# telosnetwork/plonky2_goldibear

Measured on AMD Instinct MI355X. Metric: proofs/s, higher is better.
Workload: dtype u64; 1 GPU; prove(): 2^20-row Goldilocks dummy circuit (2^19+1 NoopGates), standard_recursion_config_gl with num_challenges=3, Poseidon-12, witness in page-locked host memory, handed over every step -> proof bytes (198432 B); field=goldilocks, log_n=20, cap_height=4, proofs_in_flight_per_gpu=1, witness=in page-locked host memory, handed over every step

## Files before the change

plonky2_goldibear_amd/csrc/field_traits.hpp:

```cpp
#pragma once
#include "bb_field.hpp"
#include "gl_field.hpp"

#define GB_HD __host__ __device__ __forceinline__
#if defined(__HIP_DEVICE_COMPILE__)
#define GB_DEV_OR_HOST(dev, host) dev
#else
#define GB_DEV_OR_HOST(dev, host) host
#endif

namespace gbk {

typedef unsigned long long u64;
typedef unsigned int u32;

struct GlF {
    typedef u64 T;
    typedef gl::ext2 E;
    static constexpr u32 D = 2, H = 4, SPONGE_W = 12, ORDER_BITS = 64, TWO_ADICITY = 32, TAG = 0;
    static constexpr u64 ORDER = gl::P;
    static GB_HD T zero() { return 0; }
    static GB_HD T one() { return 1; }
    static GB_HD T enc(u64 canonical) { return canonical; }
    static GB_HD u64 dec(T x) { return x; }
    static GB_HD T reduce_word(T x) { return x >= gl::P ? x - gl::P : x; }
    static GB_HD T add(T a, T b) { return gl::add(a, b); }
    static GB_HD T sub(T a, T b) { return gl::sub(a, b); }
    static GB_HD T mul(T a, T b) { return gl::mul(a, b); }
    static GB_HD T mul_lazy(T a, T b) {
        u32 r0, r1, hl, hh;
        gl::mul_limbs(a, b, r0, r1, hl, hh);
        return gl::fold128(r0, r1, hl, hh);
    }
    static GB_HD T add_lazy(T a, T b) { return gl::add(a, b); }
    static GB_HD T cform(T c) { return gl::to_mont_slow(c); }
    static GB_HD T chain_one(u32 len) {
        constexpr unsigned __int128 R = gl::EPS;
        struct Tab { u64 v[17]; };
        constexpr Tab t = [] {
            Tab x{};
            unsigned __int128 a = 1;
            for (int i = 0; i < 17; i++) { x.v[i] = (u64)a; a = a * R % gl::P; }
            return x;
        }();
        return t.v[len];
    }
    static GB_HD T mul_chain(T acc, T f) { return gl::mul_mont_lazy(acc, f); }
    static GB_HD T mulc(T x, T c_form) { return gl::mul_mont(x, c_form); }
    typedef T Acc;
    static GB_HD Acc acc_from(T x) { return x; }
    static GB_HD void acc_mac2(Acc& a0, Acc& a1, T term, T c0, T c1) {
        a0 = add(a0, mulc(term, c0));
        a1 = add(a1, mulc(term, c1));
    }
    static GB_HD void acc_mac(Acc& a, T term, T c) { a = add(a, mulc(term, c)); }
    static GB_HD T acc_finish(Acc a) { return a; }
    static GB_HD T inv(T a) { return gl::inv(a); }
    static GB_HD T pow(T a, u64 e) { return gl::pow(a, e); }
    static GB_HD T generator() { return gl::GENERATOR; }
    static GB_HD T two_adic_generator(u32 bits) { return gl::two_adic_generator(bits); }
    static GB_HD T ext_w() { return 7; }
    static GB_HD E ezero() { return gl::e2(0); }
    static GB_HD E efrom(T x) { return gl::e2(x); }
    static GB_HD E eadd(E a, E b) { return gl::add(a, b); }
    static GB_HD E esub(E a, E b) { return gl::sub(a, b); }
    static GB_HD E emul(E a, E b) { return gl::mul(a, b); }
    static GB_HD E escale(E a, T s) { return gl::scale(a, s); }
    static GB_HD E einv(E a) { return gl::inv(a); }
    static GB_HD T coord(const E& e, u32 k) { return k ? e.c1 : e.c0; }
    static GB_HD void set_coord(E& e, u32 k, T v) { if (k) e.c1 = v; else e.c0 = v; }
};

struct bb_ext4 {
    u32 c[4];
};

struct BbF {
    typedef u32 T;
    typedef bb_ext4 E;
    static constexpr u32 D = 4, H = 8, SPONGE_W = 16, ORDER_BITS = 31, TWO_ADICITY = 27, TAG = 1;
    static constexpr u64 ORDER = bb::P;
    static constexpr u32 W_MONT = (u32)((11ull << 32) % bb::P);
    static GB_HD T zero() { return 0; }
    static GB_HD T one() { return bb::R1; }
    static GB_HD T enc(u64 canonical) { return bb::to_mont((u32)canonical); }
    static GB_HD u64 dec(T x) { return bb::from_mont(x); }
    static GB_HD T reduce_word(T x) {
        x = x >= 2 * bb::P ? x - 2 * bb::P : x;
        return x >= bb::P ? x - bb::P : x;
    }
    static GB_HD T add(T a, T b) { return bb::add(a, b); }
    static GB_HD T sub(T a, T b) { return bb::sub(a, b); }
    static GB_HD T mul(T a, T b) { return bb::mul(a, b); }
    static GB_HD T mul_lazy(T a, T b) { return bb::mul(a, b); }
    static GB_HD T add_lazy(T a, T b) { return a + b; }
    static GB_HD T cform(T c) { return c; }
    static GB_HD T mulc(T x, T c_form) { return bb::mul(x, c_form); }
    static GB_HD T chain_one(u32) { return bb::R1; }
    static GB_HD T mul_chain(T acc, T f) { return bb::mul(acc, f); }
    struct Acc {
        u64 lo;
        u32 hi;
    };
    static GB_HD Acc acc_from(T x) { return Acc{(u64)x << 32, 0u}; }
    static GB_HD void acc_mac2(Acc& a0, Acc& a1, T term, T c0, T c1) {
#if defined(__HIP_DEVICE_COMPILE__)
        u64 k0, k1;
        asm("v_mad_u64_u32 %0, %4, %6, %7, %0\n\t"
            "v_mad_u64_u32 %2, %5, %6, %8, %2\n\t"
            "s_nop 0\n\t"
            "v_addc_co_u32_e64 %1, %4, 0, %1, %4\n\t"
            "v_addc_co_u32_e64 %3, %5, 0, %3, %5"
            : "+v"(a0.lo), "+v"(a0.hi), "+v"(a1.lo), "+v"(a1.hi), "=&s"(k0), "=&s"(k1)
            : "v"(term), "s"(c0), "s"(c1));
#else
        acc_mac(a0, term, c0);
        acc_mac(a1, term, c1);
#endif
    }
    static GB_HD void acc_mac(Acc& a, T term, T c) {
        const u64 p = (u64)term * c, s = a.lo + p;
        a.hi += s < p;
        a.lo = s;
    }
    static GB_HD T acc_finish(Acc a) {
        const T top = bb::mul(a.hi, bb::R2);
        const T mid = bb::mul((u32)(a.lo >> 32), bb::R1);
        const T low = bb::reduce((u64)(u32)a.lo);
        return bb::add(bb::add(top, mid), low);
    }
    static GB_HD T inv(T a) { return bb::inv(a); }
    static GB_HD T pow(T a, u64 e) { return bb::pow(a, e); }
    static GB_HD T generator() { return bb::to_mont(bb::GENERATOR); }
    static GB_HD T two_adic_generator(u32 bits) { return bb::two_adic_generator(bits); }
    static GB_HD T ext_w() { return W_MONT; }
    static GB_HD E ezero() { return E{{0, 0, 0, 0}}; }
    static GB_HD E efrom(T x) { return E{{x, 0, 0, 0}}; }
    static GB_HD E eadd(E a, E b) { return E{{bb::add(a.c[0], b.c[0]), bb::add(a.c[1], b.c[1]), bb::add(a.c[2], b.c[2]), bb::add(a.c[3], b.c[3])}}; }
    static GB_HD E esub(E a, E b) { return E{{bb::sub(a.c[0], b.c[0]), bb::sub(a.c[1], b.c[1]), bb::sub(a.c[2], b.c[2]), bb::sub(a.c[3], b.c[3])}}; }
    static GB_HD E emul(E a, E b) {
        using bb::add; using bb::mul;
        u32 lo0 = mul(a.c[0], b.c[0]);
        u32 lo1 = add(mul(a.c[0], b.c[1]), mul(a.c[1], b.c[0]));
        u32 lo2 = add(add(mul(a.c[0], b.c[2]), mul(a.c[1], b.c[1])), mul(a.c[2], b.c[0]));
        u32 lo3 = add(add(mul(a.c[0], b.c[3]), mul(a.c[1], b.c[2])), add(mul(a.c[2], b.c[1]), mul(a.c[3], b.c[0])));
        u32 hi0 = add(add(mul(a.c[1], b.c[3]), mul(a.c[2], b.c[2])), mul(a.c[3], b.c[1]));
        u32 hi1 = add(mul(a.c[2], b.c[3]), mul(a.c[3], b.c[2]));
        u32 hi2 = mul(a.c[3], b.c[3]);
        return E{{add(lo0, mul(W_MONT, hi0)), add(lo1, mul(W_MONT, hi1)), add(lo2, mul(W_MONT, hi2)), lo3}};
    }
    static GB_HD E escale(E a, T s) { return E{{bb::mul(a.c[0], s), bb::mul(a.c[1], s), bb::mul(a.c[2], s), bb::mul(a.c[3], s)}}; }
    static __host__ __device__ inline E einv(E a) {
        using bb::add; using bb::sub; using bb::mul;
        const u32 a0 = a.c[0], a1 = a.c[1], a2 = a.c[2], a3 = a.c[3];
        u32 b2_0 = add(mul(a1, a1), mul(W_MONT, mul(a3, a3))), b2_1 = mul(add(a1, a1), a3);
        u32 c0 = sub(add(mul(a0, a0), mul(W_MONT, mul(a2, a2))), mul(W_MONT, b2_1));
        u32 c1 = sub(mul(add(a0, a0), a2), b2_0);
        u32 ninv = bb::inv(sub(mul(c0, c0), mul(W_MONT, mul(c1, c1))));
        u32 d0 = mul(c0, ninv), d1 = mul(bb::neg(c1), ninv);
        u32 ad0 = add(mul(a0, d0), mul(W_MONT, mul(a2, d1))), ad1 = add(mul(a0, d1), mul(a2, d0));
        u32 bd0 = add(mul(a1, d0), mul(W_MONT, mul(a3, d1))), bd1 = add(mul(a1, d1), mul(a3, d0));
        return E{{ad0, bb::neg(bd0), ad1, bb::neg(bd1)}};
    }
    static GB_HD T coord(const E& e, u32 k) { return e.c[k]; }
    static GB_HD void set_coord(E& e, u32 k, T v) { e.c[k] = v; }
};

template <class F>
__host__ __device__ inline typename F::E epow(typename F::E b, u64 e) {
    typename F::E r = F::efrom(F::one());
    while (e) {
        if (e & 1) r = F::emul(r, b);
        b = F::emul(b, b);
        e >>= 1;
    }
    return r;
}
template <class F>
__host__ __device__ inline bool eis_one(const typename F::E& e) {
    bool ok = F::coord(e, 0) == F::one();
    for (u32 k = 1; k < F::D; k++) ok = ok && F::coord(e, k) == F::zero();
    return ok;
}

}
```

plonky2_goldibear_amd/csrc/kernels_prover.hip:

```cpp
#include "kernels.hpp"
#include "poseidon2_bb.hpp"
#include "poseidon_gl_grouped.hpp"
#include "sponge.hpp"

namespace gbk {

__device__ __forceinline__ u32 brev32(u32 x, u32 bits) { return bits ? (__brev(x) >> (32 - bits)) : 0; }

template <class F>
__device__ __forceinline__ typename F::T pow_split(const PowTab<F>& t, u64 e) {
    typename F::T lo = t.lo[e & ((1u << t.lo_bits) - 1)];
    u64 h = e >> t.lo_bits;
    return h ? F::mul(lo, t.hi[h]) : lo;
}
template <class F>
__device__ __forceinline__ typename F::E pow_split(const ExtPowTab<F>& t, u64 e) {
    typename F::E l = t.lo[e & ((1u << t.lo_bits) - 1)];
    u64 h = e >> t.lo_bits;
    return h ? F::emul(l, t.hi[h]) : l;
}


template <class F>
__global__ __launch_bounds__(256) void k_zs_quotients(ZsParams<F> p, const typename F::T* __restrict__ witness,
                                                      const typename F::T* __restrict__ sigma, const typename F::T* __restrict__ k_is,
                                                      typename F::T* __restrict__ q, u32* __restrict__ err) {
    typedef typename F::T T;
    const u32 nb = (u32)((((size_t)1 << p.log_n) + 255) >> 8), L = blockIdx.x;
    u32 rb, ch;
    if ((nb & 7) == 0) {
        const u32 group = L / (8 * p.num_challenges), in = L % (8 * p.num_challenges);
        rb = group * 8 + (in & 7);
        ch = in >> 3;
    } else {
        rb = L % nb;
        ch = L / nb;
    }
    const u32 row = rb * 256 + threadIdx.x;
    const size_t n = (size_t)1 << p.log_n;
    if (row >= n) return;
    const T beta = p.betas[ch], gamma = p.gammas[ch];
    const T bx = F::mul(beta, pow_split(p.w_n, row));
    T N[MAX_CHUNKS], Dn[MAX_CHUNKS];
    for (u32 m = 0; m < p.nchunks; m++) {
        T np = F::one(), dp = F::one();
        const u32 j1 = min((m + 1) * p.chunk, p.num_routed);
        for (u32 j = m * p.chunk; j < j1; j++) {
            T w = witness[(size_t)j * n + row];
            const T wg = F::add(w, gamma);
            T num = F::add_lazy(wg, F::mul(bx, k_is[j]));
            T den = F::add_lazy(wg, F::mul(beta, sigma[(size_t)j * n + row]));
            np = F::mul_lazy(np, num);
            dp = F::mul_lazy(dp, den);
        }
        N[m] = np;
        Dn[m] = dp;
    }
    T pref[MAX_CHUNKS];
    T acc = F::one();
    for (u32 m = 0; m < p.nchunks; m++) {
        pref[m] = acc;
        acc = F::mul(acc, Dn[m]);
    }
    if (acc == F::zero()) {
        atomicOr(err, 1u);
        return;
    }
    T inv_run = F::inv(acc);
    for (u32 m = p.nchunks; m-- > 0;) {
        T dinv = F::mul(inv_run, pref[m]);
        inv_run = F::mul(inv_run, Dn[m]);
        q[((size_t)ch * p.nchunks + m) * n + row] = F::mul(N[m], dinv);
    }
}

template <class F>
__global__ __launch_bounds__(256) void k_zs_scan_local(ZsParams<F> p, const typename F::T* __restrict__ q,
                                                       typename F::T* __restrict__ zloc, typename F::T* __restrict__ totals) {
    typedef typename F::T T;
    __shared__ T sh[256];
    const size_t n = (size_t)1 << p.log_n;
    const u32 ch = blockIdx.y;
    const size_t row0 = (size_t)blockIdx.x * 1024 + threadIdx.x * 4;
    T r[4];
#pragma unroll
    for (int k = 0; k < 4; k++) {
        T v = F::one();
        if (row0 + k < n)
            for (u32 m = 0; m < p.nchunks; m++) v = F::mul(v, q[((size_t)ch * p.nchunks + m) * n + row0 + k]);
        r[k] = v;
    }
    T mine = F::mul(F::mul(r[0], r[1]), F::mul(r[2], r[3]));
    sh[threadIdx.x] = mine;
    __syncthreads();
    for (u32 off = 1; off < 256; off <<= 1) {
        T v = sh[threadIdx.x];
        T o = threadIdx.x >= off ? sh[threadIdx.x - off] : F::one();
        __syncthreads();
        sh[threadIdx.x] = F::mul(v, o);
        __syncthreads();
    }
    T excl = threadIdx.x ? sh[threadIdx.x - 1] : F::one();
    if (threadIdx.x == 255) totals[(size_t)ch * gridDim.x + blockIdx.x] = sh[255];
#pragma unroll
    for (int k = 0; k < 4; k++) {
        if (row0 + k < n) zloc[(size_t)ch * n + row0 + k] = excl;
        excl = F::mul(excl, r[k]);
    }
}

template <class F>
__global__ __launch_bounds__(1024) void k_zs_scan_totals(typename F::T* __restrict__ totals, u32 nblocks) {
    typedef typename F::T T;
    __shared__ T sh[1024];
    T* t = totals + (size_t)blockIdx.x * nblocks;
    const u32 C = (nblocks + 1023) / 1024, b0 = threadIdx.x * C;
    T mine = F::one();
    for (u32 k = 0; k < C; k++)
        if (b0 + k < nblocks) mine = F::mul(mine, t[b0 + k]);
    sh[threadIdx.x] = mine;
    __syncthreads();
    for (u32 off = 1; off < 1024; off <<= 1) {
        T v = sh[threadIdx.x];
        T o = threadIdx.x >= off ? sh[threadIdx.x - off] : F::one();
        __syncthreads();
        sh[threadIdx.x] = F::mul(v, o);
        __syncthreads();
    }
    T run = threadIdx.x ? sh[threadIdx.x - 1] : F::one();
    for (u32 k = 0; k < C; k++)
        if (b0 + k < nblocks) {
            const T v = t[b0 + k];
            t[b0 + k] = run;
            run = F::mul(run, v);
        }
}

template <class F>
__global__ __launch_bounds__(256) void k_zs_finalize(ZsParams<F> p, const typename F::T* __restrict__ q,
                                                     const typename F::T* __restrict__ zloc, const typename F::T* __restrict__ totals,
                                                     u32 nblocks, typename F::T* __restrict__ out) {
    typedef typename F::T T;
    const size_t n = (size_t)1 << p.log_n;
    const size_t row = (size_t)blockIdx.x * 256 + threadIdx.x;
    const u32 ch = blockIdx.y;
    if (row >= n) return;
    T z = F::mul(totals[(size_t)ch * nblocks + (row >> 10)], zloc[(size_t)ch * n + row]);
    out[(size_t)ch * n + row] = z;
    const u32 num_prods = p.nchunks - 1;
    T acc = z;
    for (u32 m = 0; m < num_prods; m++) {
        acc = F::mul(acc, q[((size_t)ch * p.nchunks + m) * n + row]);
        out[((size_t)p.num_challenges + (size_t)ch * num_prods + m) * n + row] = acc;
    }
}


#define GB_QUOTIENT_OCC(F) (sizeof(typename F::T) == 8 ? 5 : 4)
template <class F, u32 C, u32 CH, bool SLICE>
__global__ __launch_bounds__(256, GB_QUOTIENT_OCC(F)) void k_quotient(QuotientParams<F> p, const typename F::T* __restrict__ cs,
                                                  const typename F::T* __restrict__ wires, const typename F::T* __restrict__ zs,
                                                  const typename F::T* __restrict__ uni, typename F::T* __restrict__ qv) {
    typedef typename F::T T;
    const u32 lgn = p.log_n, r = p.rate_bits;
    const size_t n = (size_t)1 << lgn, N = (size_t)1 << p.stride_bits;
    const size_t j = (size_t)blockIdx.x * 256 + threadIdx.x;
    if (j >= (n << r)) return;
    const u32 CT = SLICE ? p.total_challenges : C, k0 = SLICE ? p.k0 : 0;
    const u32 cidx = (u32)(j >> lgn), jl = (u32)(j & (n - 1));
    const u32 il = brev32(jl, lgn);
    const u32 imod = brev32(cidx, r);
    const u64 i = ((u64)il << r) | imod;
    const T x = F::mul(F::generator(), pow_split(p.w_N, i));
    const size_t jn = ((size_t)cidx << lgn) | brev32((il + 1) & (u32)(n - 1), lgn);

    const u32 nr = p.num_routed, nterms = p.nterms, R = 1u << r;
    const T* betas = uni;
    const T* gammas = uni + CT;
    const T* bk = uni + 2 * CT;
    const T* zh = uni + 2 * CT + (size_t)CT * nr + (size_t)CT * nterms;
    const T* zh_inv = zh + R;
    const T* pi_hash = zh_inv + R;
    const T* apow = pi_hash + F::H + (size_t)k0 * nterms;
    if (SLICE) qv += ((size_t)k0 << r) * n;

    typename F::Acc acc[C];
#pragma unroll
    for (u32 k = 0; k < C; k++) acc[k] = F::acc_from(p.ext_gates ? qv[(((size_t)k << r) + cidx) * n + il] : F::zero());
    auto fold = [&](T term, u32 tt) {
#pragma unroll
        for (u32 k2 = 0; k2 + 1 < C; k2 += 2) F::acc_mac2(acc[k2], acc[k2 + 1], term, apow[k2 * nterms + tt], apow[(k2 + 1) * nterms + tt]);
        if (C & 1) F::acc_mac(acc[C - 1], term, apow[(C - 1) * nterms + tt]);
    };
    u32 t = 0;
    const T l0 = p.l0[j];
    const u32 num_prods = p.nchunks - 1;
    for (u32 kt0 = 0; kt0 < CT; kt0 += C) {
    auto kt = [&](u32 k) -> u32 { return SLICE ? min(kt0 + k, CT - 1) : k; };
    auto is_live = [&](u32 k) -> bool { return !SLICE || kt0 + k < CT; };
    T zk[C];
#pragma unroll
    for (u32 k = 0; k < C; k++) zk[k] = zs[(size_t)kt(k) * N + j];
#pragma unroll
    for (u32 k = 0; k < C; k++) {
        if (is_live(k)) fold(F::mul(l0, F::sub(zk[k], F::one())), kt(k));
    }
    T prev[C];
#pragma unroll
    for (u32 k = 0; k < C; k++) prev[k] = zk[k];
    for (u32 m = 0; m < p.nchunks; m++) {
        T wv[CH], sg[CH];
        const u32 w0 = m * CH;
#pragma unroll
        for (u32 q = 0; q < CH; q++) {
            const u32 w = w0 + q < nr ? w0 + q : nr - 1;
            wv[q] = wires[(size_t)w * N + j];
            sg[q] = cs[(size_t)(p.num_constants + w) * N + j];
        }
        T next[C];
#pragma unroll
        for (u32 k = 0; k < C; k++)
            next[k] = m == num_prods ? zs[(size_t)kt(k) * N + jn] : zs[((size_t)CT + (size_t)kt(k) * num_prods + m) * N + j];
        T np[C], dp[C];
        const u32 live = min(CH, nr - w0);
#pragma unroll
        for (u32 k = 0; k < C; k++) np[k] = dp[k] = F::chain_one(live);
        if (live == CH) {
#pragma unroll
            for (u32 q = 0; q < CH; q++) {
#pragma unroll
                for (u32 k = 0; k < C; k++) {
                    const T wg = F::add(wv[q], gammas[kt(k)]);
                    T num = F::add_lazy(wg, F::mulc(x, bk[kt(k) * nr + w0 + q]));
                    T den = F::add_lazy(wg, F::mulc(sg[q], betas[kt(k)]));
                    np[k] = F::mul_chain(np[k], num);
                    dp[k] = F::mul_chain(dp[k], den);
                }
            }
        } else {
#pragma unroll
            for (u32 q = 0; q < CH; q++) {
                if (q >= live) continue;
#pragma unroll
                for (u32 k = 0; k < C; k++) {
                    const T wg = F::add(wv[q], gammas[kt(k)]);
                    T num = F::add_lazy(wg, F::mulc(x, bk[kt(k) * nr + w0 + q]));
                    T den = F::add_lazy(wg, F::mulc(sg[q], betas[kt(k)]));
                    np[k] = F::mul_chain(np[k], num);
                    dp[k] = F::mul_chain(dp[k], den);
                }
            }
        }
#pragma unroll
        for (u32 k = 0; k < C; k++) {
            const T term = F::sub(F::mul(prev[k], np[k]), F::mul(next[k], dp[k]));
            if (is_live(k)) fold(term, CT + kt(k) * p.nchunks + m);
            prev[k] = next[k];
        }
    }
    }
    t = CT + CT * p.nchunks;
    if (!p.ext_gates) {
        const T s = cs[j];
        T f[3];
#pragma unroll
        for (u32 g = 0; g < 3; g++) {
            T v = F::one();
#pragma unroll
            for (u32 ii = 0; ii < 3; ii++)
                if (ii != g) v = F::mul(v, F::sub(F::enc(ii), s));
            f[g] = v;
        }
        const T f_pi = p.gate_pi == 0 ? f[0] : (p.gate_pi == 1 ? f[1] : f[2]);
        const T f_c = p.gate_constant == 0 ? f[0] : (p.gate_constant == 1 ? f[1] : f[2]);
#pragma unroll
        for (u32 cj = 0; cj < F::H; cj++, t++) {
            const T wv = wires[(size_t)cj * N + j];
            T term = F::mul(f_pi, F::sub(wv, pi_hash[cj]));
            if (cj < p.num_gate_consts) {
                const T kc = cs[(size_t)(p.num_selectors + cj) * N + j];
                term = F::add(term, F::mul(f_c, F::sub(kc, wv)));
            }
            fold(term, t);
        }
    }
#pragma unroll
    for (u32 k = 0; k < C; k++) qv[(((size_t)k << r) + cidx) * n + il] = F::mul(F::acc_finish(acc[k]), zh_inv[imod]);
}

template <class F>
__global__ __launch_bounds__(256) void k_l0_table(u32 log_n, u32 rate_bits, PowTab<F> w_N, const typename F::T* __restrict__ zh,
                                                  typename F::T* __restrict__ l0) {
    typedef typename F::T T;
    const size_t n = (size_t)1 << log_n, N = n << rate_bits;
    const size_t j = (size_t)blockIdx.x * 256 + threadIdx.x;
    if (j >= N) return;
    const u32 cidx = (u32)(j >> log_n), jl = (u32)(j & (n - 1));
    const u32 imod = brev32(cidx, rate_bits);
    const u64 i = ((u64)brev32(jl, log_n) << rate_bits) | imod;
    const T x = F::mul(F::generator(), pow_split(w_N, i));
    l0[j] = F::mul(zh[imod], F::inv(F::mul(F::enc((u64)n), F::sub(x, F::one()))));
}

template <class F>
__global__ __launch_bounds__(256) void k_quotient_combine(u32 log_n, u32 rate_bits, const typename F::T* __restrict__ a,
                                                          const typename F::T* __restrict__ mat, CosetPow<F> inv_shift,
                                                          typename F::T* __restrict__ out) {
    typedef typename F::T T;
    const size_t n = (size_t)1 << log_n;
    const u32 R = 1u << rate_bits;
    const size_t t = (size_t)blockIdx.x * 256 + threadIdx.x;
    const u32 k = blockIdx.y;
    if (t >= n) return;
    T v[MAX_RATE];
    for (u32 c = 0; c < R; c++) {
        T s = inv_shift.lo[(size_t)c * inv_shift.nlo + (t & (inv_shift.nlo - 1))];
        size_t h = t / inv_shift.nlo;
        if (h) s = F::mul(s, inv_shift.hi[(size_t)c * inv_shift.nhi + h]);
        v[c] = F::mul(a[((size_t)k * R + c) * n + t], s);
    }
    for (u32 m = 0; m < R; m++) {
        T acc = F::zero();
        for (u32 c = 0; c < R; c++) acc = F::add(acc, F::mul(v[c], mat[m * R + c]));
        out[((size_t)k * R + m) * n + t] = acc;
    }
}


template <class F>
__global__ __launch_bounds__(256) void k_ext_powtabs(ExtPowJobs<F> jobs) {
    const ExtPowJob<F>& J = jobs.j[blockIdx.y];
    const u32 t = blockIdx.x * 256 + threadIdx.x;
    if (t < J.nlo) J.lo[t] = epow<F>(J.z, t);
    else if (t - J.nlo < J.nhi) J.hi[t - J.nlo] = epow<F>(J.z, (u64)(t - J.nlo) << 10);
}

template <class F>
__global__ __launch_bounds__(256) void k_ext_pow_tables(ExtPowTables<F> z, size_t n) {
    size_t t = (size_t)blockIdx.x * 256 + threadIdx.x;
    if (t < n) z.table[blockIdx.y][t] = pow_split(z.z[blockIdx.y], t);
}

template <class F>
__device__ __forceinline__ typename F::E block_reduce_add(typename F::E v, typename F::E* sh) {
    sh[threadIdx.x] = v;
    __syncthreads();
    for (u32 off = 128; off > 0; off >>= 1) {
        if (threadIdx.x < off) sh[threadIdx.x] = F::eadd(sh[threadIdx.x], sh[threadIdx.x + off]);
        __syncthreads();
    }
    typename F::E r = sh[0];
    __syncthreads();
    return r;
}

template <class F>
__global__ __launch_bounds__(256) void k_eval_partial(EvalJobs<F> jobs, size_t n, typename F::E* __restrict__ partial) {
    typedef typename F::E E;
    __shared__ E sh[256];
    u32 col = blockIdx.y, j = 0;
    while (col >= jobs.j[j].ncols) col -= jobs.j[j++].ncols;
    const typename F::T* c = jobs.j[j].coeffs + (size_t)col * n;
    const E* ztab = jobs.j[j].ztab;
    const size_t base = (size_t)blockIdx.x * 4096;
    E acc = F::ezero();
    for (u32 k = 0; k < 16; k++) {
        size_t t = base + k * 256 + threadIdx.x;
        if (t < n) acc = F::eadd(acc, F::escale(ztab[t], c[t]));
    }
    E r = block_reduce_add<F>(acc, sh);
    if (threadIdx.x == 0) partial[(size_t)blockIdx.y * gridDim.x + blockIdx.x] = r;
}
template <class F>
__global__ __launch_bounds__(256) void k_eval_final(const typename F::E* __restrict__ partial, u32 nchunks,
                                                    typename F::E* __restrict__ out) {
    typedef typename F::E E;
    __shared__ E sh[256];
    E acc = F::ezero();
    for (u32 k = threadIdx.x; k < nchunks; k += 256) acc = F::eadd(acc, partial[(size_t)blockIdx.x * nchunks + k]);
    E r = block_reduce_add<F>(acc, sh);
    if (threadIdx.x == 0) out[blockIdx.x] = r;
}


template <class F>
__global__ __launch_bounds__(256) void k_reduce_polys(PolyGroups<F> g, size_t n, const typename F::E* __restrict__ apow,
                                                      typename F::E* __restrict__ comp) {
    size_t t = (size_t)blockIdx.x * 256 + threadIdx.x;
    if (t >= n) return;
    typename F::E acc = F::ezero();
    u32 jj = 0;
    for (u32 o = 0; o < g.ngroups; o++) {
        const typename F::T* base = g.ptr[o];
        for (u32 j = 0; j < g.ncols[o]; j++, jj++) acc = F::eadd(acc, F::escale(apow[jj], base[(size_t)j * n + t]));
    }
    comp[t] = acc;
}

template <class F>
struct alignas(16) ColVec {
    static constexpr u32 V = 16 / sizeof(typename F::T);
    typename F::T v[V];
};
template <class F>
__global__ __launch_bounds__(256) void k_reduce_batches(const ReduceRun<F>* __restrict__ runs, u32 nruns, u32 nslots, size_t n,
                                                        const typename F::E* __restrict__ apow, typename F::E* __restrict__ comp) {
    typedef typename F::T T;
    typedef typename F::E E;
    constexpr u32 V = ColVec<F>::V;
    const bool whole = n % V == 0;
    for (size_t t0 = ((size_t)blockIdx.x * 256 + threadIdx.x) * V; t0 < n; t0 += (size_t)gridDim.x * 256 * V) {
        E acc[REDUCE_SLOTS][V];
#pragma unroll
        for (u32 s = 0; s < REDUCE_SLOTS; s++)
#pragma unroll
            for (u32 e = 0; e < V; e++) acc[s][e] = F::ezero();
        auto load = [&](const T* col) {
            ColVec<F> c;
            if (whole) {
                typedef u32 v4u __attribute__((ext_vector_type(4)));
                const v4u w = *(const __attribute__((address_space(1))) v4u*)(col + t0);
                __builtin_memcpy(&c, &w, sizeof c);
            } else {
#pragma unroll
                for (u32 e = 0; e < V; e++) c.v[e] = t0 + e < n ? col[t0 + e] : F::zero();
            }
            return c;
        };
        auto mac = [&](const ReduceRun<F>& R, u32 k, const ColVec<F>& c) {
#pragma unroll
            for (u32 s = 0; s < REDUCE_SLOTS; s++)
                if (R.apow0[s] != REDUCE_ABSENT) {
                    const E a = apow[R.apow0[s] + k];
#pragma unroll
                    for (u32 e = 0; e < V; e++) acc[s][e] = F::eadd(acc[s][e], F::escale(a, c.v[e]));
                }
        };
        for (u32 r = 0; r < nruns; r++) {
            const ReduceRun<F> R = runs[r];
            u32 k = 0;
            for (; k + 4 <= R.ncols; k += 4) {
                const T* col = R.base + (size_t)k * n;
                const ColVec<F> c0 = load(col), c1 = load(col + n), c2 = load(col + 2 * n), c3 = load(col + 3 * n);
                mac(R, k, c0);
                mac(R, k + 1, c1);
                mac(R, k + 2, c2);
                mac(R, k + 3, c3);
            }
            for (; k < R.ncols; k++) mac(R, k, load(R.base + (size_t)k * n));
        }
#pragma unroll
        for (u32 s = 0; s < REDUCE_SLOTS; s++)
            if (s < nslots) {
#pragma unroll
                for (u32 e = 0; e < V; e++)
                    if (t0 + e < n) comp[(size_t)s * n + t0 + e] = acc[s][e];
            }
    }
}

template <class F>
__global__ __launch_bounds__(256) void k_divide_local(const typename F::E* __restrict__ comp, size_t n, ExtPowTab<F> z,
                                                      typename F::E* __restrict__ sloc, typename F::E* __restrict__ totals) {
    typedef typename F::E E;
    __shared__ E sh[256];
    const size_t u0 = (size_t)blockIdx.x * 1024 + threadIdx.x * 4;
    E w[4];
#pragma unroll
    for (int k = 0; k < 4; k++) w[k] = u0 + k < n ? F::emul(comp[u0 + k], pow_split(z, u0 + k)) : F::ezero();
    E mine = F::eadd(F::eadd(w[0], w[1]), F::eadd(w[2], w[3]));
    sh[threadIdx.x] = mine;
    __syncthreads();
    for (u32 off = 1; off < 256; off <<= 1) {
        E v = sh[threadIdx.x];
        E o = threadIdx.x + off < 256 ? sh[threadIdx.x + off] : F::ezero();
        __syncthreads();
        sh[threadIdx.x] = F::eadd(v, o);
        __syncthreads();
    }
    if (threadIdx.x == 0) totals[blockIdx.x] = sh[0];
    E run = threadIdx.x + 1 < 256 ? sh[threadIdx.x + 1] : F::ezero();
#pragma unroll
    for (int k = 3; k >= 0; k--) {
        run = F::eadd(run, w[k]);
        if (u0 + k < n) sloc[u0 + k] = run;
    }
}
template <class F>
__global__ __launch_bounds__(1024) void k_divide_totals(typename F::E* __restrict__ totals, u32 nblocks) {
    typedef typename F::E E;
    __shared__ E sh[1024];
    const u32 C = (nblocks + 1023) / 1024, b0 = threadIdx.x * C;
    E mine = F::ezero();
    for (u32 k = 0; k < C; k++)
        if (b0 + k < nblocks) mine = F::eadd(mine, totals[b0 + k]);
    sh[threadIdx.x] = mine;
    __syncthreads();
    for (u32 off = 1; off < 1024; off <<= 1) {
        E v = sh[threadIdx.x];
        E o = threadIdx.x + off < 1024 ? sh[threadIdx.x + off] : F::ezero();
        __syncthreads();
        sh[threadIdx.x] = F::eadd(v, o);
        __syncthreads();
    }
    E run = threadIdx.x + 1 < 1024 ? sh[threadIdx.x + 1] : F::ezero();
    for (u32 k = C; k-- > 0;)
        if (b0 + k < nblocks) {
            const E v = totals[b0 + k];
            totals[b0 + k] = run;
            run = F::eadd(run, v);
        }
}
template <class F>
__global__ __launch_bounds__(256) void k_divide_apply(const typename F::E* __restrict__ sloc, const typename F::E* __restrict__ totals,
                                                      size_t n, ExtPowTab<F> zinv, typename F::E shift, int first,
                                                      typename F::E* __restrict__ final_poly) {
    typedef typename F::E E;
    size_t t = (size_t)blockIdx.x * 256 + threadIdx.x;
    if (t >= n) return;
    E q = F::ezero();
    if (t + 1 < n) {
        size_t u = t + 1;
        E S = F::eadd(sloc[u], totals[u >> 10]);
        q = F::emul(S, pow_split(zinv, u));
    }
    final_poly[t] = first ? q : F::eadd(F::emul(final_poly[t], shift), q);
}
template <class F>
__global__ __launch_bounds__(256) void k_ext_split(const typename F::E* __restrict__ src, size_t n, typename F::T* __restrict__ dst) {
    size_t t = (size_t)blockIdx.x * 256 + threadIdx.x;
    if (t >= n) return;
    typename F::E v = src[t];
#pragma unroll
    for (u32 k = 0; k < F::D; k++) dst[(size_t)k * n + t] = F::coord(v, k);
}



template <class F>
__global__ __launch_bounds__(256) void k_fri_leaves(const typename F::T* __restrict__ vals, size_t len, u32 arity_bits,
                                                    u64 num_leaves, typename F::T* __restrict__ out) {
    typedef typename F::T T;
    constexpr u32 D = F::D, H = F::H, PER = 8 / D;
    const u64 m0 = (u64)blockIdx.x * 256 + threadIdx.x;
    const bool live = m0 < num_leaves;
    const u64 m = live ? m0 : num_leaves - 1;
    const u32 arity = 1u << arity_bits;
    const T* a = vals + (m << arity_bits);
    T* o = out + (size_t)H * m;
    if (D * arity <= H) {
        if (!live) return;
        for (u32 i = 0; i < H; i++) o[i] = 0;
        for (u32 k = 0; k < arity; k++)
            for (u32 d = 0; d < D; d++) o[D * k + d] = (T)F::dec(a[(size_t)d * len + k]);
        return;
    }
    __shared__ poseidon_gl::v4i sponge_lds[Sponge<F>::LDS_V4];
    Sponge<F> sp;
    sp.init(sponge_lds);
    for (u32 k0 = 0; k0 < arity; k0 += PER) {
#pragma unroll
        for (u32 k = 0; k < PER; k++)
            if (k0 + k < arity) {
#pragma unroll
                for (u32 d = 0; d < D; d++) sp.s[D * k + d] = a[(size_t)d * len + k0 + k];
            }
        sp.permute();
    }
    if (!live) return;
#pragma unroll
    for (u32 i = 0; i < H; i++) o[i] = sp.out(i);
}

template <class F>
__global__ __launch_bounds__(256) void k_fri_fold(const typename F::T* __restrict__ in, size_t in_len, u32 arity_bits,
                                                  typename F::E beta, typename F::T* __restrict__ out) {
    typedef typename F::E E;
    const size_t out_len = in_len >> arity_bits;
    size_t m = (size_t)blockIdx.x * 256 + threadIdx.x;
    if (m >= out_len) return;
    const u32 arity = 1u << arity_bits;
    E acc = F::ezero();
    for (u32 t = arity; t-- > 0;) {
        size_t idx = (m << arity_bits) + t;
        E v = F::ezero();
#pragma unroll
        for (u32 k = 0; k < F::D; k++) F::set_coord(v, k, in[(size_t)k * in_len + idx]);
        acc = F::eadd(F::emul(acc, beta), v);
    }
#pragma unroll
    for (u32 k = 0; k < F::D; k++) out[(size_t)k * out_len + m] = F::coord(acc, k);
}

template <class F>
__global__ __launch_bounds__(256) void k_pow_grind(PowState<F> st, u64 start, u64 count, u32 min_leading_zeros,
                                                   u64* __restrict__ result) {
    const u64 g0 = (u64)blockIdx.x * 256 + threadIdx.x;
    const bool live = g0 < count;
    const u64 g = live ? g0 : count - 1;
    u64 cand = start + g;
    __shared__ poseidon_gl::v4i sponge_lds[Sponge<F>::LDS_V4];
    Sponge<F> sp;
    sp.init(sponge_lds);
#pragma unroll
    for (int i = 0; i < (int)F::SPONGE_W; i++) sp.set_canonical(i, (u32)i == st.pos ? (typename F::T)cand : st.s[i]);
    sp.permute();
    u64 resp = sp.out(7);
    u32 lz = resp ? (u32)__clzll((long long)resp) : 64;
    if (live && lz >= min_leading_zeros) atomicMin(result, cand);
}


template <class F, bool INLINE>
__global__ __launch_bounds__(256) void k_query_gather(QueryJobs<F> jobs, QueryIdx inl, const u64* __restrict__ idx, u32 nidx,
                                                      typename F::T* __restrict__ out) {
    constexpr u32 H = F::H, D = F::D;
    const QueryJob<F>& J = jobs.j[blockIdx.y];
    u32 g = blockIdx.x * blockDim.x + threadIdx.x;
    const u32 nrow = nidx * J.width;
    const bool row = g < nrow;
    if (!row) g -= nrow;
    if (!row && g >= nidx * J.layers * H) return;
    const u32 q = row ? g / J.width : (g / H) / J.layers;
    u64 x = 0;
    if (INLINE) {
#pragma unroll
        for (u32 i = 0; i < QUERY_IDX_INLINE; i++) x = q == i ? inl.v[i] : x;
    } else {
        x = idx[q];
    }
    const u64 leaf = x >> J.shift;
    if (row) {
        const u32 e = g % J.width;
        const size_t src = J.fri ? (size_t)(e % D) * J.stride + (leaf << J.arity_bits) + e / D : (size_t)e * J.stride + leaf;
        out[J.out + g] = (typename F::T)F::dec(J.vals[src]);
        return;
    }
    const u32 e = g % H, i = (g / H) % J.layers;
    const u64 N = (u64)1 << J.log_leaves;
    const u64 off = 2 * N - ((2 * N) >> i);
    out[J.out + nrow + g] = J.levels[H * (off + ((leaf >> i) ^ 1)) + e];
}


static inline u32 nblk(size_t n, u32 bs) { return (u32)((n + bs - 1) / bs); }

template <class F>
void zs_partial_products(const ZsParams<F>& p, const typename F::T* witness, const typename F::T* sigma, const typename F::T* k_is,
                         typename F::T* q_tmp, typename F::T* zloc_tmp, typename F::T* totals_tmp, u32* err, typename F::T* out, hipStream_t st) {
    const size_t n = (size_t)1 << p.log_n;
    const u32 nb1024 = nblk(n, 1024);
    hipLaunchKernelGGL(k_zs_quotients<F>, dim3(nblk(n, 256) * p.num_challenges), dim3(256), 0, st, p, witness, sigma, k_is, q_tmp, err);
    hipLaunchKernelGGL(k_zs_scan_local<F>, dim3(nb1024, p.num_challenges), dim3(256), 0, st, p, q_tmp, zloc_tmp, totals_tmp);
    hipLaunchKernelGGL(k_zs_scan_totals<F>, dim3(p.num_challenges), dim3(1024), 0, st, totals_tmp, nb1024);
    hipLaunchKernelGGL(k_zs_finalize<F>, dim3(nblk(n, 256), p.num_challenges), dim3(256), 0, st, p, q_tmp, zloc_tmp, totals_tmp,
                       nb1024, out);
}

#define GB_Q(FF, CC, HH, SL) hipLaunchKernelGGL((k_quotient<FF, CC, HH, SL>), grid, block, 0, st, q, cs, wires, zs, uniforms, qv)
template <class F, u32 CH>
static bool quotient_slice(QuotientParams<F> q, u32 width, bool slice, const typename F::T* cs, const typename F::T* wires,
                           const typename F::T* zs, const typename F::T* uniforms, typename F::T* qv, dim3 grid, dim3 block, hipStream_t st) {
    q.num_challenges = width;
#define GB_QW(W) case W: if (slice) GB_Q(F, W, CH, true); else GB_Q(F, W, CH, false); return true
    if constexpr (F::TAG == 0) {
        switch (width) {
            GB_QW(1);
            GB_QW(2);
            case 3: if constexpr (CH == 8) { if (slice) GB_Q(F, 3, CH, true); else GB_Q(F, 3, CH, false); return true; } else return false;
            case 4: if constexpr (CH == 8) { if (slice) GB_Q(F, 4, CH, true); else GB_Q(F, 4, CH, false); return true; } else return false;
            default: return false;
        }
    } else if constexpr (CH == 8) {
        if (slice) switch (width) {
            case 5: GB_Q(F, 5, CH, true); return true;
            case 6: GB_Q(F, 6, CH, true); return true;
            case 7: GB_Q(F, 7, CH, true); return true;
            case 8: GB_Q(F, 8, CH, true); return true;
            default: return false;
        }
        switch (width) {
            case 4: GB_Q(F, 4, CH, false); return true;
            case 5: GB_Q(F, 5, CH, false); return true;
            case 6: GB_Q(F, 6, CH, false); return true;
            case 7: GB_Q(F, 7, CH, false); return true;
            case 8: GB_Q(F, 8, CH, false); return true;
            case 9: GB_Q(F, 9, CH, false); return true;
            case 10: GB_Q(F, 10, CH, false); return true;
            default: return false;
        }
    } else {
        switch (width) {
            GB_QW(4);
            GB_QW(5);
            GB_QW(6);
            GB_QW(7);
            GB_QW(8);
            default: return false;
        }
    }
#undef GB_QW
}
#undef GB_Q
static inline u32 quotient_gl_wmax(u32 chunk) { return chunk == 8 ? 4 : 2; }
static inline u32 quotient_bb_wmax(u32 chunk) { return chunk == 8 ? 10 : 8; }
template <class F>
bool quotient_values(const QuotientParams<F>& p, const typename F::T* cs, const typename F::T* wires, const typename F::T* zs,
                     const typename F::T* uniforms, typename F::T* qv, hipStream_t st) {
    const size_t NQ = (size_t)1 << (p.log_n + p.rate_bits);
    const dim3 grid(nblk(NQ, 256)), block(256);
    u32 widths[MAX_CHALLENGES];
    const u32 ns = challenge_slices(F::TAG, quotient_gl_wmax(p.chunk), p.num_challenges, widths, quotient_bb_wmax(p.chunk));
    if (!ns || !quotient_shape_supported(F::TAG, p.chunk, p.num_challenges)) return false;
    QuotientParams<F> q = p;
    q.total_challenges = p.num_challenges;
    q.k0 = 0;
    for (u32 i = 0; i < ns; q.k0 += widths[i], i++) {
        bool ok;
        switch (p.chunk) {
            case 2: ok = quotient_slice<F, 2>(q, widths[i], ns > 1, cs, wires, zs, uniforms, qv, grid, block, st); break;
            case 4: ok = quotient_slice<F, 4>(q, widths[i], ns > 1, cs, wires, zs, uniforms, qv, grid, block, st); break;
            case 8: ok = quotient_slice<F, 8>(q, widths[i], ns > 1, cs, wires, zs, uniforms, qv, grid, block, st); break;
            case 16: ok = quotient_slice<F, 16>(q, widths[i], ns > 1, cs, wires, zs, uniforms, qv, grid, block, st); break;
            default: ok = false;
        }
        if (!ok) return false;
    }
    return true;
}
template bool quotient_values<GlF>(const QuotientParams<GlF>&, const u64*, const u64*, const u64*, const u64*, u64*, hipStream_t);
template bool quotient_values<BbF>(const QuotientParams<BbF>&, const u32*, const u32*, const u32*, const u32*, u32*, hipStream_t);
bool quotient_shape_supported(u32 field, u32 chunk, u32 num_challenges) {
    u32 widths[MAX_CHALLENGES];
    if (num_challenges == 0 || num_challenges > MAX_CHALLENGES) return false;
    if (chunk != 2 && chunk != 4 && chunk != 8 && chunk != 16) return false;
    return challenge_slices(field, quotient_gl_wmax(chunk), num_challenges, widths, quotient_bb_wmax(chunk)) != 0;
}

template <class F>
void l0_table(u32 log_n, u32 rate_bits, const PowTab<F>& w_N, const typename F::T* zh, typename F::T* l0, hipStream_t st) {
    const size_t N = (size_t)1 << (log_n + rate_bits);
    hipLaunchKernelGGL(k_l0_table<F>, dim3(nblk(N, 256)), dim3(256), 0, st, log_n, rate_bits, w_N, zh, l0);
}

template <class F>
void quotient_combine(u32 log_n, u32 rate_bits, u32 num_challenges, const typename F::T* a, const typename F::T* mat,
                      const CosetPow<F>& inv_shift, typename F::T* out, hipStream_t st) {
    const size_t n = (size_t)1 << log_n;
    hipLaunchKernelGGL(k_quotient_combine<F>, dim3(nblk(n, 256), num_challenges), dim3(256), 0, st, log_n, rate_bits, a, mat,
                       inv_shift, out);
}

template <class F>
void ext_powtabs(const ExtPowJobs<F>& jobs, u32 njobs, hipStream_t st) {
    u32 most = 0;
    for (u32 j = 0; j < njobs; j++) most = std::max(most, jobs.j[j].nlo + jobs.j[j].nhi);
    if (most) hipLaunchKernelGGL(k_ext_powtabs<F>, dim3(nblk(most, 256), njobs), dim3(256), 0, st, jobs);
}

template <class F>
void ext_pow_tables(const ExtPowTables<F>& z, u32 count, size_t n, hipStream_t st) {
    if (count && n) hipLaunchKernelGGL(k_ext_pow_tables<F>, dim3(nblk(n, 256), count), dim3(256), 0, st, z, n);
}

template <class F>
void eval_columns(const EvalJobs<F>& jobs, u32 njobs, size_t n, typename F::E* partial_tmp, typename F::E* out, hipStream_t st) {
    u32 total = 0;
    for (u32 j = 0; j < njobs; j++) total += jobs.j[j].ncols;
    if (!total) return;
    const u32 nch = nblk(n, 4096);
    hipLaunchKernelGGL(k_eval_partial<F>, dim3(nch, total), dim3(256), 0, st, jobs, n, partial_tmp);
    hipLaunchKernelGGL(k_eval_final<F>, dim3(total), dim3(256), 0, st, partial_tmp, nch, out);
}

template <class F>
void reduce_polys(const PolyGroups<F>& g, size_t n, const typename F::E* apow, typename F::E* comp, hipStream_t st) {
    hipLaunchKernelGGL(k_reduce_polys<F>, dim3(nblk(n, 256)), dim3(256), 0, st, g, n, apow, comp);
}

template <class F>
void reduce_batches(const ReduceRun<F>* runs_dev, u32 nruns, u32 nslots, size_t n, const typename F::E* apow, typename F::E* comp,
                    hipStream_t st) {
    const u32 blocks = std::min<u32>(nblk(nblk(n, ColVec<F>::V), 256), 2048u);
    hipLaunchKernelGGL(k_reduce_batches<F>, dim3(blocks), dim3(256), 0, st, runs_dev, nruns, nslots, n, apow, comp);
}

template <class F>
void divide_by_linear_accumulate(const typename F::E* comp, size_t n, const ExtPowTab<F>& z, const ExtPowTab<F>& zinv,
                                 typename F::E shift, int first, typename F::E* sloc_tmp, typename F::E* totals_tmp,
                                 typename F::E* final_poly, hipStream_t st) {
    const u32 nb = nblk(n, 1024);
    hipLaunchKernelGGL(k_divide_local<F>, dim3(nb), dim3(256), 0, st, comp, n, z, sloc_tmp, totals_tmp);
    hipLaunchKernelGGL(k_divide_totals<F>, dim3(1), dim3(1024), 0, st, totals_tmp, nb);
    hipLaunchKernelGGL(k_divide_apply<F>, dim3(nblk(n, 256)), dim3(256), 0, st, sloc_tmp, totals_tmp, n, zinv, shift, first,
                       final_poly);
}

template <class F>
void ext_split(const typename F::E* src, size_t n, typename F::T* dst, hipStream_t st) {
    hipLaunchKernelGGL(k_ext_split<F>, dim3(nblk(n, 256)), dim3(256), 0, st, src, n, dst);
}

template <class F>
void fri_leaves(const typename F::T* vals, size_t len, u32 arity_bits, u64 num_leaves, typename F::T* out, hipStream_t st) {
    if constexpr (F::TAG == 0)
        if (gl_fri_leaves_coop(vals, len, arity_bits, num_leaves, out, st)) return;
    if constexpr (F::TAG == 1)
        if (bb_fri_leaves_coop(vals, len, arity_bits, num_leaves, out, st)) return;
    hipLaunchKernelGGL(k_fri_leaves<F>, dim3(nblk(num_leaves, 256)), dim3(256), 0, st, vals, len, arity_bits, num_leaves, out);
}

template <class F>
void fri_fold(const typename F::T* in, size_t in_len, u32 arity_bits, typename F::E beta, typename F::T* out, hipStream_t st) {
    hipLaunchKernelGGL(k_fri_fold<F>, dim3(nblk(in_len >> arity_bits, 256)), dim3(256), 0, st, in, in_len, arity_bits, beta, out);
}

template <class F>
void pow_grind(const PowState<F>& s, u64 start, u64 count, u32 min_lz, u64* result, hipStream_t st) {
    hipLaunchKernelGGL(k_pow_grind<F>, dim3(nblk(count, 256)), dim3(256), 0, st, s, start, count, min_lz, result);
}

template <class F>
void query_gather(const QueryJobs<F>& jobs, u32 njobs, const u64* idx_host, const u64* idx_dev, u32 nidx, typename F::T* out, hipStream_t st) {
    size_t most = 0;
    for (u32 j = 0; j < njobs; j++) most = std::max(most, (size_t)nidx * (jobs.j[j].width + (size_t)jobs.j[j].layers * F::H));
    if (!most || !njobs) return;
    QueryIdx inl{};
    if (nidx <= QUERY_IDX_INLINE) {
        std::copy(idx_host, idx_host + nidx, inl.v);
        hipLaunchKernelGGL((k_query_gather<F, true>), dim3(nblk(most, 256), njobs), dim3(256), 0, st, jobs, inl, idx_dev, nidx, out);
    } else {
        hipLaunchKernelGGL((k_query_gather<F, false>), dim3(nblk(most, 256), njobs), dim3(256), 0, st, jobs, inl, idx_dev, nidx, out);
    }
}

#define GB_INSTANTIATE(F)                                                                                                           \
    template void zs_partial_products<F>(const ZsParams<F>&, const F::T*, const F::T*, const F::T*, F::T*, F::T*, F::T*, u32*, F::T*,  \
                                         hipStream_t);                                                                              \
    template void quotient_combine<F>(u32, u32, u32, const F::T*, const F::T*, const CosetPow<F>&, F::T*, hipStream_t);             \
    template void l0_table<F>(u32, u32, const PowTab<F>&, const F::T*, F::T*, hipStream_t);                                         \
    template void ext_powtabs<F>(const ExtPowJobs<F>&, u32, hipStream_t);                                                           \
    template void ext_pow_tables<F>(const ExtPowTables<F>&, u32, size_t, hipStream_t);                                              \
    template void eval_columns<F>(const EvalJobs<F>&, u32, size_t, F::E*, F::E*, hipStream_t);                                      \
    template void reduce_polys<F>(const PolyGroups<F>&, size_t, const F::E*, F::E*, hipStream_t);                                   \
    template void reduce_batches<F>(const ReduceRun<F>*, u32, u32, size_t, const F::E*, F::E*, hipStream_t);                        \
    template void divide_by_linear_accumulate<F>(const F::E*, size_t, const ExtPowTab<F>&, const ExtPowTab<F>&, F::E, int, F::E*,   \
                                                 F::E*, F::E*, hipStream_t);                                                        \
    template void ext_split<F>(const F::E*, size_t, F::T*, hipStream_t);                                                            \
    template void fri_leaves<F>(const F::T*, size_t, u32, u64, F::T*, hipStream_t);                                                 \
    template void fri_fold<F>(const F::T*, size_t, u32, F::E, F::T*, hipStream_t);                                                  \
    template void pow_grind<F>(const PowState<F>&, u64, u64, u32, u64*, hipStream_t);                                               \
    template void query_gather<F>(const QueryJobs<F>&, u32, const u64*, const u64*, u32, F::T*, hipStream_t);
GB_INSTANTIATE(GlF)
GB_INSTANTIATE(BbF)
#undef GB_INSTANTIATE

}
```

Baseline: 10.70 proofs/s.

## Process two quotient leaves per thread sharing the coset point and vector loads

Adds a quotient kernel path in which each thread evaluates two leaves whose domain points differ only in sign (il and il+n/2). The coset-point exponentiation and the x·k_i products are then shared, with a subtraction used for the negated point. All column reads become paired 128-bit loads. The path is enabled for Goldilocks with up to 3 challenges and chunk ≤8, and launches half the grid. In exchange it roughly doubles register pressure, lowers the occupancy hint, and adds alignment guards that make the slice launcher fail otherwise.

```diff
diff --git a/plonky2_goldibear_amd/csrc/field_traits.hpp b/plonky2_goldibear_amd/csrc/field_traits.hpp
--- a/plonky2_goldibear_amd/csrc/field_traits.hpp
+++ b/plonky2_goldibear_amd/csrc/field_traits.hpp
@@ -33,6 +33,7 @@
         return gl::fold128(r0, r1, hl, hh);
     }
     static GB_HD T add_lazy(T a, T b) { return gl::add(a, b); }
+    static GB_HD T sub_lazy(T a, T b) { return gl::sub(a, b); }
     static GB_HD T cform(T c) { return gl::to_mont_slow(c); }
     static GB_HD T chain_one(u32 len) {
         constexpr unsigned __int128 R = gl::EPS;
@@ -94,6 +95,7 @@
     static GB_HD T mul(T a, T b) { return bb::mul(a, b); }
     static GB_HD T mul_lazy(T a, T b) { return bb::mul(a, b); }
     static GB_HD T add_lazy(T a, T b) { return a + b; }
+    static GB_HD T sub_lazy(T a, T b) { return a + (bb::P - b); }
     static GB_HD T cform(T c) { return c; }
     static GB_HD T mulc(T x, T c_form) { return bb::mul(x, c_form); }
     static GB_HD T chain_one(u32) { return bb::R1; }
diff --git a/plonky2_goldibear_amd/csrc/kernels_prover.hip b/plonky2_goldibear_amd/csrc/kernels_prover.hip
--- a/plonky2_goldibear_amd/csrc/kernels_prover.hip
+++ b/plonky2_goldibear_amd/csrc/kernels_prover.hip
@@ -156,11 +156,10 @@
 }
 
 
-#define GB_QUOTIENT_OCC(F) (sizeof(typename F::T) == 8 ? 5 : 4)
 template <class F, u32 C, u32 CH, bool SLICE>
-__global__ __launch_bounds__(256, GB_QUOTIENT_OCC(F)) void k_quotient(QuotientParams<F> p, const typename F::T* __restrict__ cs,
-                                                  const typename F::T* __restrict__ wires, const typename F::T* __restrict__ zs,
-                                                  const typename F::T* __restrict__ uni, typename F::T* __restrict__ qv) {
+__device__ __forceinline__ void quotient_leaf(const QuotientParams<F>& p, const typename F::T* __restrict__ cs,
+                                              const typename F::T* __restrict__ wires, const typename F::T* __restrict__ zs,
+                                              const typename F::T* __restrict__ uni, typename F::T* __restrict__ qv) {
     typedef typename F::T T;
     const u32 lgn = p.log_n, r = p.rate_bits;
     const size_t n = (size_t)1 << lgn, N = (size_t)1 << p.stride_bits;
@@ -286,6 +285,186 @@
     }
 #pragma unroll
     for (u32 k = 0; k < C; k++) qv[(((size_t)k << r) + cidx) * n + il] = F::mul(F::acc_finish(acc[k]), zh_inv[imod]);
+}
+
+template <class F>
+__device__ __forceinline__ void load_pair(const typename F::T* col, typename F::T (&v)[2]) {
+    typedef u32 W __attribute__((ext_vector_type(2 * sizeof(typename F::T) / 4)));
+    const W w = *(const __attribute__((address_space(1))) W*)col;
+    __builtin_memcpy(v, &w, sizeof v);
+}
+
+template <class F, u32 C, u32 CH, bool SLICE>
+__device__ __forceinline__ void quotient_pair(const QuotientParams<F>& p, const typename F::T* __restrict__ cs,
+                                              const typename F::T* __restrict__ wires, const typename F::T* __restrict__ zs,
+                                              const typename F::T* __restrict__ uni, typename F::T* __restrict__ qv) {
+    typedef typename F::T T;
+    constexpr u32 LV = 2;
+    const u32 lgn = p.log_n, r = p.rate_bits;
+    const size_t n = (size_t)1 << lgn, N = (size_t)1 << p.stride_bits;
+    const size_t j = ((size_t)blockIdx.x * 256 + threadIdx.x) * LV;
+    if (j >= (n << r)) return;
+    const u32 CT = SLICE ? p.total_challenges : C, k0 = SLICE ? p.k0 : 0;
+    const u32 cidx = (u32)(j >> lgn), jl = (u32)(j & (n - 1));
+    const u32 il0 = brev32(jl, lgn);
+    const u32 il[LV] = {il0, il0 + (u32)(n >> 1)};
+    const u32 imod = brev32(cidx, r);
+    const u64 i = ((u64)il0 << r) | imod;
+    const T x = F::mul(F::generator(), pow_split(p.w_N, i));
+    size_t jn[LV];
+#pragma unroll
+    for (u32 e = 0; e < LV; e++) jn[e] = ((size_t)cidx << lgn) | brev32((il[e] + 1) & (u32)(n - 1), lgn);
+
+    const u32 nr = p.num_routed, nterms = p.nterms, R = 1u << r;
+    const T* betas = uni;
+    const T* gammas = uni + CT;
+    const T* bk = uni + 2 * CT;
+    const T* zh = uni + 2 * CT + (size_t)CT * nr + (size_t)CT * nterms;
+    const T* zh_inv = zh + R;
+    const T* pi_hash = zh_inv + R;
+    const T* apow = pi_hash + F::H + (size_t)k0 * nterms;
+    if (SLICE) qv += ((size_t)k0 << r) * n;
+
+    typename F::Acc acc[LV][C];
+#pragma unroll
+    for (u32 e = 0; e < LV; e++)
+#pragma unroll
+        for (u32 k = 0; k < C; k++) acc[e][k] = F::acc_from(p.ext_gates ? qv[(((size_t)k << r) + cidx) * n + il[e]] : F::zero());
+    auto fold = [&](const T (&term)[LV], u32 tt) {
+#pragma unroll
+        for (u32 e = 0; e < LV; e++) {
+#pragma unroll
+            for (u32 k2 = 0; k2 + 1 < C; k2 += 2)
+                F::acc_mac2(acc[e][k2], acc[e][k2 + 1], term[e], apow[k2 * nterms + tt], apow[(k2 + 1) * nterms + tt]);
+            if (C & 1) F::acc_mac(acc[e][C - 1], term[e], apow[(C - 1) * nterms + tt]);
+        }
+    };
+    u32 t = 0;
+    T l0[LV];
+    load_pair<F>(p.l0 + j, l0);
+    const u32 num_prods = p.nchunks - 1;
+    for (u32 kt0 = 0; kt0 < CT; kt0 += C) {
+    auto kt = [&](u32 k) -> u32 { return SLICE ? min(kt0 + k, CT - 1) : k; };
+    auto is_live = [&](u32 k) -> bool { return !SLICE || kt0 + k < CT; };
+    T zk[C][LV];
+#pragma unroll
+    for (u32 k = 0; k < C; k++) load_pair<F>(zs + (size_t)kt(k) * N + j, zk[k]);
+#pragma unroll
+    for (u32 k = 0; k < C; k++) {
+        T term[LV];
+#pragma unroll
+        for (u32 e = 0; e < LV; e++) term[e] = F::mul(l0[e], F::sub(zk[k][e], F::one()));
+        if (is_live(k)) fold(term, kt(k));
+    }
+    T prev[C][LV];
+#pragma unroll
+    for (u32 k = 0; k < C; k++)
+#pragma unroll
+        for (u32 e = 0; e < LV; e++) prev[k][e] = zk[k][e];
+    for (u32 m = 0; m < p.nchunks; m++) {
+        T wv[CH][LV], sg[CH][LV];
+        const u32 w0 = m * CH;
+#pragma unroll
+        for (u32 q = 0; q < CH; q++) {
+            const u32 w = w0 + q < nr ? w0 + q : nr - 1;
+            load_pair<F>(wires + (size_t)w * N + j, wv[q]);
+            load_pair<F>(cs + (size_t)(p.num_constants + w) * N + j, sg[q]);
+        }
+        T next[C][LV];
+#pragma unroll
+        for (u32 k = 0; k < C; k++) {
+            if (m == num_prods) {
+#pragma unroll
+                for (u32 e = 0; e < LV; e++) next[k][e] = zs[(size_t)kt(k) * N + jn[e]];
+            } else {
+                load_pair<F>(zs + ((size_t)CT + (size_t)kt(k) * num_prods + m) * N + j, next[k]);
+            }
+        }
+        T np[C][LV], dp[C][LV];
+        const u32 live = min(CH, nr - w0);
+#pragma unroll
+        for (u32 k = 0; k < C; k++)
+#pragma unroll
+            for (u32 e = 0; e < LV; e++) np[k][e] = dp[k][e] = F::chain_one(live);
+        auto wire = [&](u32 q) {
+#pragma unroll
+            for (u32 k = 0; k < C; k++) {
+                const T xb = F::mulc(x, bk[kt(k) * nr + w0 + q]);
+#pragma unroll
+                for (u32 e = 0; e < LV; e++) {
+                    const T wg = F::add(wv[q][e], gammas[kt(k)]);
+                    T num = e ? F::sub_lazy(wg, xb) : F::add_lazy(wg, xb);
+                    T den = F::add_lazy(wg, F::mulc(sg[q][e], betas[kt(k)]));
+                    np[k][e] = F::mul_chain(np[k][e], num);
+                    dp[k][e] = F::mul_chain(dp[k][e], den);
+                }
+            }
+        };
+        if (live == CH) {
+#pragma unroll
+            for (u32 q = 0; q < CH; q++) wire(q);
+        } else {
+#pragma unroll
+            for (u32 q = 0; q < CH; q++)
+                if (q < live) wire(q);
+        }
+#pragma unroll
+        for (u32 k = 0; k < C; k++) {
+            T term[LV];
+#pragma unroll
+            for (u32 e = 0; e < LV; e++) term[e] = F::sub(F::mul(prev[k][e], np[k][e]), F::mul(next[k][e], dp[k][e]));
+            if (is_live(k)) fold(term, CT + kt(k) * p.nchunks + m);
+#pragma unroll
+            for (u32 e = 0; e < LV; e++) prev[k][e] = next[k][e];
+        }
+    }
+    }
+    t = CT + CT * p.nchunks;
+    if (!p.ext_gates) {
+        T s[LV];
+        load_pair<F>(cs + j, s);
+        T f_pi[LV], f_c[LV];
+#pragma unroll
+        for (u32 e = 0; e < LV; e++) {
+            T f[3];
+#pragma unroll
+            for (u32 g = 0; g < 3; g++) {
+                T v = F::one();
+#pragma unroll
+                for (u32 ii = 0; ii < 3; ii++)
+                    if (ii != g) v = F::mul(v, F::sub(F::enc(ii), s[e]));
+                f[g] = v;
+            }
+            f_pi[e] = p.gate_pi == 0 ? f[0] : (p.gate_pi == 1 ? f[1] : f[2]);
+            f_c[e] = p.gate_constant == 0 ? f[0] : (p.gate_constant == 1 ? f[1] : f[2]);
+        }
+#pragma unroll
+        for (u32 cj = 0; cj < F::H; cj++, t++) {
+            T wv[LV], kc[LV], term[LV];
+            load_pair<F>(wires + (size_t)cj * N + j, wv);
+            if (cj < p.num_gate_consts) load_pair<F>(cs + (size_t)(p.num_selectors + cj) * N + j, kc);
+#pragma unroll
+            for (u32 e = 0; e < LV; e++) {
+                term[e] = F::mul(f_pi[e], F::sub(wv[e], pi_hash[cj]));
+                if (cj < p.num_gate_consts) term[e] = F::add(term[e], F::mul(f_c[e], F::sub(kc[e], wv[e])));
+            }
+            fold(term, t);
+        }
+    }
+#pragma unroll
+    for (u32 e = 0; e < LV; e++)
+#pragma unroll
+        for (u32 k = 0; k < C; k++) qv[(((size_t)k << r) + cidx) * n + il[e]] = F::mul(F::acc_finish(acc[e][k]), zh_inv[imod]);
+}
+
+#define GB_QUOTIENT_LEAVES(F, C, CH) (sizeof(typename F::T) == 8 && C <= 3 && CH <= 8 ? 2 : 1)
+#define GB_QUOTIENT_OCC(F, C, CH) (GB_QUOTIENT_LEAVES(F, C, CH) == 2 ? 3 : sizeof(typename F::T) == 8 ? 5 : 4)
+template <class F, u32 C, u32 CH, bool SLICE>
+__global__ __launch_bounds__(256, GB_QUOTIENT_OCC(F, C, CH)) void k_quotient(QuotientParams<F> p, const typename F::T* __restrict__ cs,
+                                                  const typename F::T* __restrict__ wires, const typename F::T* __restrict__ zs,
+                                                  const typename F::T* __restrict__ uni, typename F::T* __restrict__ qv) {
+    if constexpr (GB_QUOTIENT_LEAVES(F, C, CH) == 2) quotient_pair<F, C, CH, SLICE>(p, cs, wires, zs, uni, qv);
+    else quotient_leaf<F, C, CH, SLICE>(p, cs, wires, zs, uni, qv);
 }
 
 template <class F>
@@ -657,10 +836,15 @@
                        nb1024, out);
 }
 
-#define GB_Q(FF, CC, HH, SL) hipLaunchKernelGGL((k_quotient<FF, CC, HH, SL>), grid, block, 0, st, q, cs, wires, zs, uniforms, qv)
+#define GB_Q(FF, CC, HH, SL)                                                                                                  \
+    hipLaunchKernelGGL((k_quotient<FF, CC, HH, SL>), dim3((leaf_grid.x + GB_QUOTIENT_LEAVES(FF, CC, HH) - 1) / GB_QUOTIENT_LEAVES(FF, CC, HH)), \
+                       block, 0, st, q, cs, wires, zs, uniforms, qv)
 template <class F, u32 CH>
 static bool quotient_slice(QuotientParams<F> q, u32 width, bool slice, const typename F::T* cs, const typename F::T* wires,
-                           const typename F::T* zs, const typename F::T* uniforms, typename F::T* qv, dim3 grid, dim3 block, hipStream_t st) {
+                           const typename F::T* zs, const typename F::T* uniforms, typename F::T* qv, dim3 leaf_grid, dim3 block, hipStream_t st) {
+    if (q.log_n < 1 || q.stride_bits < 1 ||
+        (((uintptr_t)cs | (uintptr_t)wires | (uintptr_t)zs | (uintptr_t)q.l0) & (2 * sizeof(typename F::T) - 1)))
+        return false;
     q.num_challenges = width;
 #define GB_QW(W) case W: if (slice) GB_Q(F, W, CH, true); else GB_Q(F, W, CH, false); return true
     if constexpr (F::TAG == 0) {
```

Measured after the change: 10.77 proofs/s (median of 6 runs). About the same (+0.7%).
